# astroHaoPeng/gp_algos

Hardware: NVIDIA B200
Metric: MLE objective+gradient evals/sec at n=8192 D=8 (FP64) (higher is better)
Workload: dtype f64

## Files before the change

### gp_algos_b200/csrc/gpk_chol.cu

```cuda
#include "gpk_internal.cuh"

#include <stdlib.h>

namespace {

constexpr int NB = GPK_TILE;

struct Ctx {
    gpk_handle h;
    int64_t ld;
    int keep_L;
    int* info;
    int batch;
    int64_t sM;
    int64_t sT;
    int side_base;
};

int side_min() {
    static int v = -1;
    if (v < 0) { const char* e = getenv("GPK_SIDE_MIN"); v = e ? atoi(e) : 256; }
    return v;
}

// ... 254 lines not shown
                g.Q = Li + b1 + (int64_t)bk * N; g.ldq = N; g.q_kcontig = 0;
                g.D = rhsB + b1; g.ldd = N; g.Cin = g.D; g.ldc = N;
                g.R = rhsM; g.S = N - b1; g.K = sk; g.alpha = -1.0; g.beta = 1.0;
                rc = gpk_gemm(h, g);
                if (rc) return rc;
            }
        }
    }
    cudaEvent_t e1 = next_event(h), e2 = next_event(h);
    GPK_CUDA(h, cudaEventRecord(e1, S));
    GPK_CUDA(h, cudaStreamWaitEvent(M, e1, 0));
    GPK_CUDA(h, cudaEventRecord(e2, S1));
    GPK_CUDA(h, cudaStreamWaitEvent(M, e2, 0));
    if (rhsB) {
        cudaEvent_t e3 = next_event(h);
        GPK_CUDA(h, cudaEventRecord(e3, R));
        GPK_CUDA(h, cudaStreamWaitEvent(M, e3, 0));
    }
    tr.dump();
    return GPK_OK;
}

}

size_t gpk_chol_scratch_doubles(int N) {
    const size_t rec = rec_scratch_doubles(N);
    const size_t pipe = rec_scratch_doubles(pipe_nb()) + (size_t)pipe_nb() * N;
    const size_t fact = rec_scratch_doubles(potrf_nb_max());
    const size_t m = rec > pipe ? rec : pipe;
    return m > fact ? m : fact;
}

int gpk_potrf_inv_pipelined(gpk_handle h, double* A, double* Li, double* Kinv, double* T, int N, int keep_L, int* info_dev,
                            cudaEvent_t* kinv_done) {
    const int nbk = pipe_nb();
    const int nt = (N + nbk - 1) / nbk;
    auto bs = [&](int k) { return k * nbk < N ? k * nbk : N; };
    GPK_CUDA(h, cudaMemsetAsync(info_dev, 0, sizeof(int), h->stream));
    Ctx c{h, N, keep_L, info_dev, 1, (int64_t)N * N, 0, 0};
    double* Tdiag = T;
    double* Trow = T + rec_scratch_doubles(nbk);
    cudaStream_t M = h->stream, S = h->pipe[0], S2 = h->pipe[1], S3 = h->pipe[2];
    cudaEvent_t ev = next_event(h);
    GPK_CUDA(h, cudaEventRecord(ev, M));
    GPK_CUDA(h, cudaStreamWaitEvent(S, ev, 0));
    GPK_CUDA(h, cudaStreamWaitEvent(S2, ev, 0));
    if (Kinv) GPK_CUDA(h, cudaStreamWaitEvent(S3, ev, 0));
    cudaEvent_t evGcol_prev = nullptr;
    cudaEvent_t evLi = nullptr;
    int rc;
    Trace tr;
    tr.start(M);
    for (int k = 0; k < nt; ++k) {
        const int bk = bs(k), sk = bs(k + 1) - bk;
        rc = potrf_inv_rec(c, A + bk + (int64_t)bk * N, Li + bk + (int64_t)bk * N, Tdiag, sk, bk, 0);
        if (rc) return rc;
        cudaEvent_t evF = next_event(h);
        GPK_CUDA(h, cudaEventRecord(evF, M));
        tr.mark(M, "M:F", k);
        if (k + 1 < nt) {
            const int b1 = bs(k + 1), s1 = bs(k + 2) - b1;
            rc = stage_panel(h, A, Li, N, bk, sk, b1, N, keep_L);
            if (rc) return rc;
            cudaEvent_t evE = next_event(h);
            GPK_CUDA(h, cudaEventRecord(evE, M));
            if (evGcol_prev) GPK_CUDA(h, cudaStreamWaitEvent(M, evGcol_prev, 0));
            tr.mark(M, "M:P", k);
            rc = stage_update(h, A, Li, N, bk, sk, b1, s1, b1, N - b1, 1);
            if (rc) return rc;
            tr.mark(M, "M:Ucol", k);
            evGcol_prev = nullptr;
            if (k + 2 < nt) {
                GPK_CUDA(h, cudaStreamWaitEvent(S, evE, 0));
                StreamSwap sw(h, S);
                const int b2 = bs(k + 2), s2 = bs(k + 3) - b2;
                rc = stage_update(h, A, Li, N, bk, sk, b2, s2, b2, N - b2, 1);
                if (rc) return rc;
                evGcol_prev = next_event(h);
                GPK_CUDA(h, cudaEventRecord(evGcol_prev, S));
                if (k + 3 < nt) {
                    const int b3 = bs(k + 3);
                    rc = stage_update(h, A, Li, N, bk, sk, b3, N - b3, b3, N - b3, 1);
                    if (rc) return rc;
                }
                tr.mark(S, "S:U", k);
// ... 138 lines not shown
```

### gp_algos_b200/csrc/gpk_cov.cu

```cuda
#include "gpk_internal.cuh"

#include <stdarg.h>

namespace {

constexpr int CT = 64;
constexpr int DC = 8;
constexpr int TLD = CT + 1;

enum { MODE_SYM_FULL = 0, MODE_SYM_LOWER_PAD = 1, MODE_CROSS = 2 };

struct CovArgs {
    const double* X1; int64_t ldx1; int m;
    const double* X2; int64_t ldx2; int n;
    double* K; int64_t ldk;
    int mp, np;
    int64_t strideX1, strideX2, strideK;
    const ProblemParams* pp;
    CovParams cp;
};

__device__ __forceinline__ void store2(double* p, double a, double b, bool ok0, bool ok1) {
    if (ok0 && ok1 && ((reinterpret_cast<uintptr_t>(p) & 15) == 0)) {
        *reinterpret_cast<double2*>(p) = make_double2(a, b);
    } else {
        if (ok0) p[0] = a;
        if (ok1) p[1] = b;
    }
}

template <int MODE, int KIND>
__global__ void __launch_bounds__(256) cov_se_ard_kernel(const CovArgs a0) {
    struct View { const double* X1; const double* X2; double* K; int64_t ldx1, ldx2, ldk; int m, n, mp, np; const CovParams& cp; };
    const int64_t bz = blockIdx.z;
    const View a = {a0.X1 + bz * a0.strideX1, a0.X2 + bz * a0.strideX2, a0.K + bz * a0.strideK, a0.ldx1, a0.ldx2, a0.ldk,
                    a0.m, a0.n, a0.mp, a0.np, a0.pp ? a0.pp[bz].cp : a0.cp};
    __shared__ double xi[DC][CT];
    __shared__ double xj[DC][CT];
    __shared__ double tbuf[(MODE == MODE_SYM_FULL) ? CT * TLD : 1];

    const int bi = blockIdx.x, bj = blockIdx.y;
    if (MODE == MODE_SYM_FULL && bj > bi) return;
    if (MODE == MODE_SYM_LOWER_PAD && (bj >> 1) > (bi >> 1)) return;
    const int i0 = bi * CT, j0 = bj * CT;
    const int tid = threadIdx.x, tx = tid & 31, ty = tid >> 5;
    const int D = a.cp.D;

    double r[2][8];
#pragma unroll
    for (int q = 0; q < 2; ++q)
#pragma unroll
        for (int b = 0; b < 8; ++b) r[q][b] = 0.0;

    for (int d0 = 0; d0 < D; d0 += DC) {
        const int dc = min(DC, D - d0);
        __syncthreads();
        for (int e = tid; e < dc * CT; e += 256) {
            const int d = e / CT, l = e % CT;
            const int gi = i0 + l, gj = j0 + l;
            xi[d][l] = (gi < a.m) ? a.X1[gi + (int64_t)(d0 + d) * a.ldx1] : 0.0;
            xj[d][l] = (gj < a.n) ? a.X2[gj + (int64_t)(d0 + d) * a.ldx2] : 0.0;
        }
        __syncthreads();
        for (int d = 0; d < dc; ++d) {
            const double inv = a.cp.inv_ls2[d0 + d];
            const double x0 = xi[d][2 * tx], x1 = xi[d][2 * tx + 1];
#pragma unroll
            for (int b = 0; b < 8; ++b) {
                const double xv = xj[d][ty + 8 * b];
                const double f0 = __dsub_rn(x0, xv), f1 = __dsub_rn(x1, xv);
                if (KIND == GPK_KERNEL_CO2) {
                    r[0][b] = f0; r[1][b] = f1;
                } else {
                    r[0][b] = __dadd_rn(r[0][b], __dmul_rn(__dmul_rn(f0, inv), f0));
                    r[1][b] = __dadd_rn(r[1][b], __dmul_rn(__dmul_rn(f1, inv), f1));
                }
            }
        }
    }

    const int gi0 = i0 + 2 * tx;
#pragma unroll
    for (int b = 0; b < 8; ++b) {
        const int gj = j0 + ty + 8 * b;
        double v[2];
#pragma unroll
        for (int q = 0; q < 2; ++q) {
            const int gi = gi0 + q;
            double val;
            if (KIND == GPK_KERNEL_CO2) {
                Co2Terms t;
                val = co2_value(a.cp.inv_ls2, r[q][b], t);
            } else {
                val = __dmul_rn(a.cp.sf2, exp(__dmul_rn(-0.5, r[q][b])));
            }
            if (MODE != MODE_CROSS && gi == gj) {
                val = __dadd_rn(val, a.cp.sn2);
                if (a.cp.extra_diag != 0.0) val = __dadd_rn(val, a.cp.extra_diag);
            }
            if (gi >= a.m || gj >= a.n) val = (MODE == MODE_SYM_LOWER_PAD && gi == gj) ? 1.0 : 0.0;
            v[q] = val;
        }
        store2(a.K + gi0 + (int64_t)gj * a.ldk, v[0], v[1], gi0 < a.mp && gj < a.np, gi0 + 1 < a.mp && gj < a.np);
        if (MODE == MODE_SYM_FULL) {
            tbuf[(2 * tx) * TLD + ty + 8 * b] = v[0];
            tbuf[(2 * tx + 1) * TLD + ty + 8 * b] = v[1];
        }
    }
    if (MODE == MODE_SYM_FULL && bi != bj) {
        __syncthreads();
        const int jl0 = 2 * tx;
#pragma unroll
        for (int b = 0; b < 8; ++b) {
            const int il = ty + 8 * b;
            const int grow = j0 + jl0, gcol = i0 + il;
            store2(a.K + grow + (int64_t)gcol * a.ldk, tbuf[il * TLD + jl0], tbuf[il * TLD + jl0 + 1],
                   grow < a.n && gcol < a.m, grow + 1 < a.n && gcol < a.m);
        }
    }
}

__global__ void cov_deriv_kernel(int param_num, const double* X, int n, int64_t ldx, CovParams cp, double sf, double sn,
                                 double ls_d, double* dK, int64_t ldk) {
    const int i = blockIdx.y * blockDim.x + threadIdx.x;
    const int j = blockIdx.x;
    if (i >= n || j >= n) return;
    const int D = cp.D;
    if (cp.kind == GPK_KERNEL_CO2) {
        Co2Terms t;
        double dk[GPK_CO2_NPARAMS];
        co2_value(cp.inv_ls2, __dsub_rn(X[i], X[j]), t);
        co2_derivs(cp.inv_ls2, t, dk);
        dk[10] = (i == j) ? 2 * cp.inv_ls2[10] : 0.0;
        dK[i + (int64_t)j * ldk] = dk[param_num - 1];
        return;
    }
// ... 33 lines not shown
        out->gscale[1 + d] = 0.5 * (sf * sf) / (l * l * l);
    }
    out->gscale[D + 1] = sn;
    return GPK_OK;
}

int gpk_make_cov_params(gpk_handle h, const double* theta, int D, int has_sigma_noise, double sigma_noise, CovParams* out) {
    if (D < 1 || D > GPK_MAX_D) return gpk_set_error(h, GPK_EINVAL, "feature dimension D=%d outside 1..%d", D, GPK_MAX_D);
    memset(out, 0, sizeof(*out));
    out->D = D;
    out->kind = h ? h->kernel_family : GPK_KERNEL_SE_ARD;
    if (out->kind == GPK_KERNEL_CO2) {
        if (D != 1) return gpk_set_error(h, GPK_EINVAL, "requirement failed: This kernel is applicable only for 1D objects");
        double* par = out->inv_ls2;
        for (int p = 0; p < GPK_CO2_NPARAMS; ++p) par[p] = theta[p];
        par[11] = pow(theta[1], -3); par[12] = pow(theta[3], -3); par[13] = pow(theta[4], -3); par[14] = pow(theta[6], -3);
        par[15] = pow(theta[9], -3);
        out->sf2 = ((theta[0] * theta[0] + theta[2] * theta[2]) + theta[5] * theta[5]) + theta[8] * theta[8];
        out->sn2 = theta[10] * theta[10];
        out->extra_diag = has_sigma_noise ? sigma_noise : 0.0;
        return GPK_OK;
    }
    out->sf2 = theta[0] * theta[0];
    out->sn2 = theta[D + 1] * theta[D + 1];
    out->extra_diag = has_sigma_noise ? sigma_noise : 0.0;
    for (int d = 0; d < D; ++d) out->inv_ls2[d] = 1.0 / (theta[1 + d] * theta[1 + d]);
    return GPK_OK;
}

int gpk_cov_sym_full(gpk_handle h, const double* dX, int n, int64_t ldx, const CovParams& cp, double* dK, int64_t ldk) {
    if (n <= 0) return GPK_OK;
    CovArgs a;
    a.X1 = dX; a.ldx1 = ldx; a.m = n; a.X2 = dX; a.ldx2 = ldx; a.n = n; a.K = dK; a.ldk = ldk; a.mp = n; a.np = n; a.cp = cp;
    a.strideX1 = a.strideX2 = a.strideK = 0; a.pp = nullptr;
    const int t = (n + CT - 1) / CT;
    if (cp.kind == GPK_KERNEL_CO2) cov_se_ard_kernel<MODE_SYM_FULL, GPK_KERNEL_CO2><<<dim3(t, t), 256, 0, h->stream>>>(a);
    else cov_se_ard_kernel<MODE_SYM_FULL, GPK_KERNEL_SE_ARD><<<dim3(t, t), 256, 0, h->stream>>>(a);
    GPK_LAUNCH_CHECK(h);
    return GPK_OK;
}

int gpk_cov_sym_lower_padded(gpk_handle h, const double* dX, int n, int64_t ldx, const CovParams& cp, double* dK, int N,
                             int batch, int64_t strideX, const ProblemParams* pp_dev) {
    CovArgs a;
    a.X1 = dX; a.ldx1 = ldx; a.m = n; a.X2 = dX; a.ldx2 = ldx; a.n = n; a.K = dK; a.ldk = N; a.mp = N; a.np = N; a.cp = cp;
    a.strideX1 = a.strideX2 = strideX; a.strideK = (int64_t)N * N; a.pp = pp_dev;
    const int t = N / CT;
    if (cp.kind == GPK_KERNEL_CO2) cov_se_ard_kernel<MODE_SYM_LOWER_PAD, GPK_KERNEL_CO2><<<dim3(t, t, batch), 256, 0, h->stream>>>(a);
    else cov_se_ard_kernel<MODE_SYM_LOWER_PAD, GPK_KERNEL_SE_ARD><<<dim3(t, t, batch), 256, 0, h->stream>>>(a);
    GPK_LAUNCH_CHECK(h);
    return GPK_OK;
}

int gpk_cov_cross(gpk_handle h, const double* dX1, int m, int64_t ldx1, const double* dX2, int n, int64_t ldx2,
                  const CovParams& cp, double* dK, int64_t ldk, int mp, int np, int batch, int64_t strideX1, int64_t strideX2,
                  int64_t strideK, const ProblemParams* pp_dev) {
    if (mp < m) mp = m;
    if (np < n) np = n;
    if (mp <= 0 || np <= 0) return GPK_OK;
    CovArgs a;
    a.X1 = dX1; a.ldx1 = ldx1; a.m = m; a.X2 = dX2; a.ldx2 = ldx2; a.n = n; a.K = dK; a.ldk = ldk; a.mp = mp; a.np = np; a.cp = cp;
    a.strideX1 = strideX1; a.strideX2 = strideX2; a.strideK = strideK; a.pp = pp_dev;
    const dim3 grid((mp + CT - 1) / CT, (np + CT - 1) / CT, batch);
    if (cp.kind == GPK_KERNEL_CO2) cov_se_ard_kernel<MODE_CROSS, GPK_KERNEL_CO2><<<grid, 256, 0, h->stream>>>(a);
    else cov_se_ard_kernel<MODE_CROSS, GPK_KERNEL_SE_ARD><<<grid, 256, 0, h->stream>>>(a);
    GPK_LAUNCH_CHECK(h);
    return GPK_OK;
}

int gpk_cov_deriv(gpk_handle h, int param_num, const double* dX, int n, int64_t ldx, const CovParams& cp, double sf,
                  double sn, const double* ls_host, double* dK, int64_t ldk) {
    if (n <= 0) return GPK_OK;
    const double ls_d = (param_num >= 2 && param_num < cp.D + 2) ? ls_host[param_num - 2] : 1.0;
    cov_deriv_kernel<<<dim3(n, (n + 127) / 128), 128, 0, h->stream>>>(param_num, dX, n, ldx, cp, sf, sn, ls_d, dK, ldk);
    GPK_LAUNCH_CHECK(h);
    return GPK_OK;
}
```

### gp_algos_b200/csrc/gpk_gp.cu

```cuda
#include "gpk_internal.cuh"

#include <stdlib.h>

#include <new>

namespace {

#define ARENA_OR_FAIL(ptr, type, h, which, bytes)           \
    type ptr = (type)gpk_arena((h), (which), (bytes));      \
    if (!ptr) return GPK_ENOMEM

size_t batch_budget_bytes() {
    static size_t v = 0;
    if (!v) {
        const char* e = getenv("GPK_BATCH_GB");
        v = (size_t)((e ? atof(e) : 48.0) * (1ull << 30));
    }
    return v;
}

struct Work {
    int N, B;
    double *A, *Li, *T, *ypad, *z, *alpha, *scratch;
    size_t sT, sScratch;
// ... 23 lines not shown
    double* m = (double*)gpk_arena(h, ARENA_MISC, (size_t)B * ((size_t)3 * N + sScr) * sizeof(double));
    w->pp_dev = (ProblemParams*)gpk_arena(h, ARENA_PP, (size_t)B * sizeof(ProblemParams));
    w->info_dev = (int*)gpk_arena(h, ARENA_INFO, (size_t)B * sizeof(int));
    if (!w->A || !w->Li || !w->T || !m || !w->pp_dev || !w->info_dev) return GPK_ENOMEM;
    w->ypad = m;
    w->z = m + (size_t)B * N;
    w->alpha = m + (size_t)2 * B * N;
    w->scratch = m + (size_t)3 * B * N;
    return GPK_OK;
}

int stage_params(gpk_handle h, const double* thetas, int D, int has_s, double s, int B, ProblemParams* dev, ProblemParams* first) {
    const size_t bytes = (size_t)B * sizeof(ProblemParams);
    if (h->pp_host_bytes < bytes) {
        free(h->pp_host);
        h->pp_host = malloc(bytes);
        h->pp_host_bytes = h->pp_host ? bytes : 0;
        if (!h->pp_host) return gpk_set_error(h, GPK_ENOMEM, "host allocation failed");
    }
    ProblemParams* hp = (ProblemParams*)h->pp_host;
    for (int b = 0; b < B; ++b) {
        int rc = gpk_make_problem_params(h, thetas + (size_t)b * gpk_theta_len(h, D), D, has_s, s, &hp[b]);
        if (rc) return rc;
    }
    *first = hp[0];
    if (B > 1) {
        GPK_CUDA(h, cudaMemcpyAsync(dev, hp, bytes, cudaMemcpyHostToDevice, h->stream));
    }
    return GPK_OK;
}

int fit_core(gpk_handle h, const Work& w, int B, const double* dX, int n, int D, int64_t ldx, int64_t strideX, const double* dy,
             const ProblemParams& pp0, int keep_L, double* Li, double* alpha, double* ll_dev, int64_t ll_stride, int* info_dev,
             double* Kinv = nullptr, cudaEvent_t* kinv_done = nullptr, bool params_on_device = false) {
    const ProblemParams* ppd = (B > 1 || params_on_device) ? w.pp_dev : nullptr;
    int rc = gpk_cov_sym_lower_padded(h, dX, n, ldx, pp0.cp, w.A, w.N, B, strideX, ppd);
    if (rc) return rc;
    rc = Kinv ? gpk_potrf_inv_pipelined(h, w.A, Li, Kinv, w.T, w.N, keep_L, info_dev, kinv_done)
              : gpk_potrf_inv(h, w.A, Li, w.T, w.N, keep_L, info_dev, B);
    if (rc) return rc;
    rc = gpk_pad_vector(h, w.ypad, w.N, dy, n, B);
    if (rc) return rc;
    rc = gpk_trmv_lower(h, Li, w.N, w.ypad, w.z, w.scratch, B);
    if (rc) return rc;
    rc = gpk_trmv_lower_t(h, Li, w.N, w.z, alpha, B);
    if (rc) return rc;
    return gpk_loglik(h, w.A, w.N, n, w.ypad, alpha, ll_dev, B, ll_stride);
}

int nll_grad_core(gpk_handle h, int B, const double* dX, int n, int D, int64_t ldx, int64_t strideX, const double* dy,
                  const double* thetas, int has_s, double s, int nparams, double* out_dev, int* info_dev,
                  const ProblemParams* pp_single = nullptr) {
    Work w;
    int rc = make_work(h, n, D, B, &w);
    if (rc) return rc;
    const int64_t so = nparams + 1;
    const bool on_dev = pp_single != nullptr;
    for (int b0 = 0; b0 < B; b0 += w.B) {
        const int bc = (B - b0 < w.B) ? B - b0 : w.B;
        ProblemParams pp0;
        if (on_dev) pp0 = *pp_single;
        else rc = stage_params(h, thetas + (size_t)b0 * gpk_theta_len(h, D), D, has_s, s, bc, w.pp_dev, &pp0);
        if (rc) return rc;
        const double* X = dX + b0 * strideX;
        int* info = info_dev ? info_dev + b0 : (B == 1 ? h->d_info : w.info_dev);
        double* Kinv = nullptr;
        if (nparams > 0 && gpk_use_pipelined(w.N, bc)) {
            Kinv = (double*)gpk_arena(h, ARENA_KINV, (size_t)w.N * w.N * sizeof(double));
            if (!Kinv) return GPK_ENOMEM;
        }
        cudaEvent_t kinv_done = nullptr;
        rc = fit_core(h, w, bc, X, n, D, ldx, strideX, dy + (size_t)b0 * n, pp0, 0, w.Li, w.alpha, out_dev + b0 * so, so, info, Kinv,
                      &kinv_done, on_dev);
        if (rc) return rc;
        if (kinv_done) GPK_CUDA(h, cudaStreamWaitEvent(h->stream, kinv_done, 0));
        if (nparams > 0) {
            if (!Kinv) {
                rc = gpk_lauum_lower(h, w.Li, w.A, w.N, bc);
                if (rc) return rc;
            }
            rc = gpk_grad_trace(h, Kinv ? Kinv : w.A, w.N, X, n, ldx, w.alpha, pp0, nparams, out_dev + b0 * so + 1, w.scratch, bc, strideX,
                                (bc > 1 || on_dev) ? w.pp_dev : nullptr, so);
            if (rc) return rc;
        }
    }
    return GPK_OK;
}

__global__ void store_params_kernel(const ProblemParams pp, ProblemParams* __restrict__ dst) {
    if (threadIdx.x == 0) *dst = pp;
}

int nll_grad_single(gpk_handle h, const double* dX, int n, int D, int64_t ldx, const double* dy, const double* theta, int has_s,
                    double s, int nparams, double* out_dev, int* info_dev) {
    if (!h->graph_mode) return nll_grad_core(h, 1, dX, n, D, ldx, 0, dy, theta, has_s, s, nparams, out_dev, info_dev);
    ProblemParams pp;
    int rc = gpk_make_problem_params(h, theta, D, has_s, s, &pp);
    if (rc) return rc;
    Work w;
    rc = make_work(h, n, D, 1, &w);
    if (rc) return rc;
    if (nparams > 0 && gpk_use_pipelined(w.N, 1) && !gpk_arena(h, ARENA_KINV, (size_t)w.N * w.N * sizeof(double))) return GPK_ENOMEM;
    GraphKey key;
    memset(&key, 0, sizeof(key));
    key.p[0] = dX; key.p[1] = dy; key.p[2] = out_dev; key.p[3] = info_dev;
    key.i[0] = n; key.i[1] = D; key.i[2] = nparams; key.i[3] = ldx; key.i[4] = h->kernel_family;
    store_params_kernel<<<1, 32, 0, h->stream>>>(pp, w.pp_dev);
    GPK_LAUNCH_CHECK(h);
    auto body = [&]() { return nll_grad_core(h, 1, dX, n, D, ldx, 0, dy, theta, has_s, s, nparams, out_dev, info_dev, &pp); };
    static int after = -1;
    if (after < 0) { const char* e = getenv("GPK_GRAPH_AFTER_EVAL"); after = e ? atoi(e) : 1; if (after < 1) after = 1; }
    return gpk_graph_run(h, GPK_SLOT_EVAL, key, after, body, "evaluation");
}


__global__ void __launch_bounds__(256) ucb_grad_kernel(const double* __restrict__ KsT, const double* __restrict__ U, int N, int n,
                                                       const double* __restrict__ X, int ldx, const double* __restrict__ Xs, int ms,
                                                       const double* __restrict__ alpha, const double* __restrict__ colsq,
                                                       const double* __restrict__ mean, CovParams cp, double kparam,
                                                       double* __restrict__ grad, double* __restrict__ ucb, double* __restrict__ var) {
    __shared__ double sa[256], sb[256];
    const int c = blockIdx.x, d = blockIdx.y;
    const double xd = Xs[c + (int64_t)d * ms], inv = cp.inv_ls2[d];
    const double* ks = KsT + (int64_t)c * N;
    const double* u = U + (int64_t)c * N;
    const double* xcol = X + (int64_t)d * ldx;
    double a = 0.0, b = 0.0;
    for (int i = threadIdx.x; i < n; i += 256) {
        const double g = ((xd - xcol[i]) * inv) * (-ks[i]);
        a += g * alpha[i];
        b += g * u[i];
    }
    sa[threadIdx.x] = a; sb[threadIdx.x] = b;
    __syncthreads();
    for (int s = 128; s > 0; s >>= 1) {
// ... 546 lines not shown
```

### gp_algos_b200/csrc/gpk_grad.cu

```cuda
#include "gpk_internal.cuh"

namespace {

constexpr int GT = 64;
constexpr int GC = 8;

struct GradArgs {
    const double* Kinv; int N;
    const double* X; int64_t ldx; int n;
    const double* alpha;
    double* partial;
    int64_t strideX;
    const ProblemParams* pp;
    CovParams cp;
};

__device__ __forceinline__ double block_sum(double v, double* red) {
#pragma unroll
    for (int o = 16; o > 0; o >>= 1) v += __shfl_xor_sync(0xffffffffu, v, o);
    const int w = threadIdx.x >> 5, l = threadIdx.x & 31;
    __syncthreads();
    if (l == 0) red[w] = v;
    __syncthreads();
    double s = 0.0;
    if (threadIdx.x == 0)
        for (int i = 0; i < 8; ++i) s += red[i];
    return s;
}

__global__ void __launch_bounds__(256) grad_trace_kernel(const GradArgs a) {
    extern __shared__ double sm[];
    __shared__ double red[8];
    const int64_t pb = blockIdx.y;
    const CovParams& cp = a.pp ? a.pp[pb].cp : a.cp;
    const double* Kinv = a.Kinv ? a.Kinv + pb * (int64_t)a.N * a.N : nullptr;
    const double* X = a.X + pb * a.strideX;
    const double* alpha = a.alpha + pb * a.N;
    const int D = cp.D;
    double* xi = sm;
    double* xj = sm + D * GT;
    const int t = blockIdx.x;
    int bi = (int)((sqrt(8.0 * (double)t + 1.0) - 1.0) * 0.5);
    while ((int64_t)(bi + 1) * (bi + 2) / 2 <= t) ++bi;
    while ((int64_t)bi * (bi + 1) / 2 > t) --bi;
    const int bj = t - (int)((int64_t)bi * (bi + 1) / 2);
    const int i0 = bi * GT, j0 = bj * GT;
    const int tid = threadIdx.x, tx = tid & 31, ty = tid >> 5;

    for (int e = tid; e < D * GT; e += 256) {
        const int d = e / GT, l = e % GT;
        const int gi = i0 + l, gj = j0 + l;
        xi[e] = (gi < a.n) ? X[gi + (int64_t)d * a.ldx] : 0.0;
        xj[e] = (gj < a.n) ? X[gj + (int64_t)d * a.ldx] : 0.0;
    }
    __syncthreads();

    const int gi0 = i0 + 2 * tx;
    double we[2][8];
    double wdiag = 0.0;
    {
        double r[2][8];
#pragma unroll
        for (int q = 0; q < 2; ++q)
#pragma unroll
            for (int b = 0; b < 8; ++b) r[q][b] = 0.0;
        for (int d = 0; d < D; ++d) {
            const double inv = cp.inv_ls2[d];
            const double x0 = xi[d * GT + 2 * tx], x1 = xi[d * GT + 2 * tx + 1];
#pragma unroll
            for (int b = 0; b < 8; ++b) {
                const double xv = xj[d * GT + ty + 8 * b];
                const double f0 = x0 - xv, f1 = x1 - xv;
                r[0][b] += (f0 * inv) * f0;
                r[1][b] += (f1 * inv) * f1;
            }
        }
        const double al0 = (gi0 < a.n) ? alpha[gi0] : 0.0, al1 = (gi0 + 1 < a.n) ? alpha[gi0 + 1] : 0.0;
#pragma unroll
        for (int b = 0; b < 8; ++b) {
            const int gj = j0 + ty + 8 * b;
            const double aj = (gj < a.n) ? alpha[gj] : 0.0;
            const double2 kv = Kinv ? *reinterpret_cast<const double2*>(Kinv + gi0 + (int64_t)gj * a.N) : make_double2(0.0, 0.0);
#pragma unroll
            for (int q = 0; q < 2; ++q) {
                const int gi = gi0 + q;
                const double w = (q ? al1 : al0) * aj - (q ? kv.y : kv.x);
                const bool valid = gi < a.n && gj < a.n && gi >= gj;
                const double mult = (gi == gj) ? 1.0 : 2.0;
                we[q][b] = valid ? mult * w * exp(-0.5 * r[q][b]) : 0.0;
                if (valid && gi == gj) wdiag += w;
            }
        }
    }

    double* out = a.partial + (pb * gridDim.x + blockIdx.x) * (int64_t)(D + 2);
    {
        double s = 0.0;
#pragma unroll
        for (int q = 0; q < 2; ++q)
#pragma unroll
            for (int b = 0; b < 8; ++b) s += we[q][b];
        const double ts = block_sum(s, red);
        const double tn = block_sum(wdiag, red);
        if (tid == 0) { out[0] = ts; out[D + 1] = tn; }
    }
    for (int d0 = 0; d0 < D; d0 += GC) {
        double acc[GC];
#pragma unroll
        for (int c = 0; c < GC; ++c) acc[c] = 0.0;
#pragma unroll
        for (int c = 0; c < GC; ++c) {
            const int d = d0 + c;
            if (d < D) {
                const double x0 = xi[d * GT + 2 * tx], x1 = xi[d * GT + 2 * tx + 1];
#pragma unroll
                for (int b = 0; b < 8; ++b) {
                    const double xv = xj[d * GT + ty + 8 * b];
                    const double f0 = x0 - xv, f1 = x1 - xv;
                    acc[c] += we[0][b] * (f0 * f0) + we[1][b] * (f1 * f1);
                }
            }
        }
// ... 57 lines not shown
    }
}

struct GradScale { double s[GPK_MAX_D + 2]; };
__global__ void __launch_bounds__(256) grad_finish_kernel(const double* partial, int nblocks, int np_all, int nparams,
                                                          const GradScale scale, const ProblemParams* pp, double* g,
                                                          int64_t strideOut) {
    __shared__ double sd[256];
    const int p = blockIdx.x;
    const int64_t pb = blockIdx.y;
    if (p >= nparams) return;
    partial += pb * (int64_t)nblocks * np_all;
    double s = 0.0;
    for (int b = threadIdx.x; b < nblocks; b += 256) s += partial[(int64_t)b * np_all + p];
    sd[threadIdx.x] = s;
    __syncthreads();
    for (int k = 128; k > 0; k >>= 1) {
        if (threadIdx.x < k) sd[threadIdx.x] += sd[threadIdx.x + k];
        __syncthreads();
    }
    if (threadIdx.x == 0) g[pb * strideOut + p] = (pp ? pp[pb].gscale[p] : scale.s[p]) * sd[0];
}

}

size_t gpk_grad_scratch_doubles(int N, int D) {
    const size_t tiles = (size_t)(N / GT) * (N / GT + 1) / 2;
    const size_t np = (size_t)(D + 2 > GPK_CO2_NPARAMS ? D + 2 : GPK_CO2_NPARAMS);
    return tiles * np + np;
}

int gpk_grad_trace(gpk_handle h, const double* Kinv, int N, const double* dX, int n, int64_t ldx, const double* alpha,
                   const ProblemParams& pp, int nparams, double* g_out, double* scratch, int batch, int64_t strideX,
                   const ProblemParams* pp_dev, int64_t strideOut) {
    const int D = pp.cp.D;
    const int np_all = pp.cp.kind == GPK_KERNEL_CO2 ? GPK_CO2_NPARAMS : D + 2;
    if (nparams < 0 || nparams > np_all) return gpk_set_error(h, GPK_EINVAL, "nparams=%d outside 0..%d", nparams, np_all);
    if (nparams == 0) return GPK_OK;
    const int nt = (n + GT - 1) / GT;
    const int nblocks = nt * (nt + 1) / 2;
    GradArgs a;
    a.Kinv = Kinv; a.N = N; a.X = dX; a.ldx = ldx; a.n = n; a.alpha = alpha; a.partial = scratch; a.cp = pp.cp;
    a.strideX = strideX; a.pp = pp_dev;
    const size_t smem = (size_t)2 * D * GT * sizeof(double);
    if (smem > 48 * 1024 && !(h->func_cfg & (1u << 9))) {
        GPK_CUDA(h, cudaFuncSetAttribute(grad_trace_kernel, cudaFuncAttributeMaxDynamicSharedMemorySize,
                                         (int)((size_t)2 * GPK_MAX_D * GT * sizeof(double))));
        h->func_cfg |= (1u << 9);
    }
    if (pp.cp.kind == GPK_KERNEL_CO2) grad_trace_co2_kernel<<<dim3(nblocks, batch), 256, 0, h->stream>>>(a);
    else grad_trace_kernel<<<dim3(nblocks, batch), 256, smem, h->stream>>>(a);
    GPK_LAUNCH_CHECK(h);
    GradScale sc;
    memcpy(sc.s, pp.gscale, sizeof(sc.s));
    grad_finish_kernel<<<dim3(nparams, batch), 256, 0, h->stream>>>(scratch, nblocks, np_all, nparams, sc, pp_dev, g_out, strideOut);
    GPK_LAUNCH_CHECK(h);
    return GPK_OK;
}
```

### gp_algos_b200/csrc/gpk_internal.cuh

```cuda
#pragma once
#include <cuda_runtime.h>
#include <stdint.h>
#include <stdio.h>
#include <string.h>

#include <functional>

#include "../../include/gpk.h"

#define GPK_TILE 128
#define GPK_NPIPE 3
#define GPK_NSIDE 16
#define GPK_NGROUP 4
#define GPK_NEVENTS 256

struct gpk_handle_s {
    int device;
    cudaStream_t stream;
    cudaStream_t main_stream;
    int num_sms;
    bool own_stream;
    cudaStream_t side[GPK_NSIDE];
    cudaStream_t grp[GPK_NGROUP - 1];
    cudaStream_t pipe[GPK_NPIPE];
// ... 5 lines not shown
    void* res_pinned;
    size_t res_pinned_bytes;
    int* d_info;
    int last_info;
    int64_t launches;
    unsigned func_cfg;
    void* pp_host;
    size_t pp_host_bytes;
    int graph_mode;
    unsigned arena_epoch;
    struct gpk_graph_slot* slots[3];
    struct gpk_capture_log* cap;
    int prio_main, prio_side, prio_pipe;
    int kernel_family;
    char err[512];
};
struct StreamSwap {
    gpk_handle h; cudaStream_t saved;
    StreamSwap(gpk_handle h_, cudaStream_t s) : h(h_), saved(h_->stream) { h->stream = s; }
    ~StreamSwap() { h->stream = saved; }
};
static inline cudaEvent_t next_event(gpk_handle h) { return h->evpool[h->ev_next++ % GPK_NEVENTS]; }
#define GPK_NSLOTS 3
enum { GPK_SLOT_EVAL = 0, GPK_SLOT_EP_SWEEP = 1, GPK_SLOT_POTRF = 2 };
struct GraphKey { const void* p[6]; int64_t i[6]; };
void gpk_capture_note(gpk_handle h);
void gpk_graph_drop_all(gpk_handle h);
int gpk_graph_run_impl(gpk_handle h, int slot, const GraphKey& key, int eager_calls, int (*body)(void*), void* ctx, const char* what);
template <class F>
int gpk_graph_run(gpk_handle h, int slot, const GraphKey& key, int eager_calls, F& body, const char* what) {
    return gpk_graph_run_impl(h, slot, key, eager_calls, [](void* c) { return (*static_cast<F*>(c))(); }, &body, what);
}

enum { ARENA_A = 0, ARENA_B = 1, ARENA_T = 2, ARENA_MISC = 3, ARENA_X = 4, ARENA_IO = 5, ARENA_IO2 = 6, ARENA_IO3 = 7, ARENA_PP = 8, ARENA_INFO = 9, ARENA_GEMV = 10, ARENA_KINV = 11, GPK_NARENA = 12 };

int gpk_set_error(gpk_handle h, int status, const char* fmt, ...);
void* gpk_arena(gpk_handle h, int which, size_t bytes);
int gpk_upload_matrix(gpk_handle h, double* dst, const double* src, int rows, int cols, int64_t ld);
int gpk_download_matrix(gpk_handle h, double* dst, int64_t ld, const double* src, int rows, int cols);
int gpk_finish_info(gpk_handle h);

#define GPK_CUDA(h, call)                                                                         \
    do {                                                                                          \
        cudaError_t e__ = (call);                                                                 \
        if (e__ != cudaSuccess)                                                                   \
            return gpk_set_error((h), e__ == cudaErrorMemoryAllocation ? GPK_ENOMEM : GPK_ECUDA,  \
                                 "%s failed: %s (%s:%d)", #call, cudaGetErrorString(e__), __FILE__, __LINE__); \
    } while (0)

#define GPK_LAUNCH_CHECK(h)                                                                       \
    do {                                                                                          \
        (h)->launches++;                                                                          \
        if ((h)->cap) gpk_capture_note(h);                                                        \
        cudaError_t e__ = cudaGetLastError();                                                     \
        if (e__ != cudaSuccess)                                                                   \
            return gpk_set_error((h), GPK_ECUDA, "kernel launch failed: %s (%s:%d)",              \
                                 cudaGetErrorString(e__), __FILE__, __LINE__);                    \
    } while (0)

static inline int gpk_pad(int n) { return (n + GPK_TILE - 1) / GPK_TILE * GPK_TILE; }

struct GemmDesc {
    const double* P; int64_t ldp; int64_t strideP;
    const double* Q; int64_t ldq; int64_t strideQ;
    double* D; int64_t ldd; int64_t strideD;
    const double* Cin; int64_t ldc; int64_t strideC;
    int R, S, K;
// ... 55 lines not shown
    const double first = exp(__dmul_rn(-hp8, lg));
    const double den = __dmul_rn(__dmul_rn(__dmul_rn(__dmul_rn(__dmul_rn(2.0, hp7), hp7), hp8), hp8), t.p1);
    const double second = __dadd_rn(-lg, __dmul_rn(hp8, t.sq) / den);
    dk[7] = __dmul_rn(__dmul_rn(__dmul_rn(hp6, hp6), first), second);
    dk[8] = __dmul_rn(2.0, t.k4) / hp9;
    dk[9] = __dmul_rn(__dmul_rn(t.k4, t.sq), par[15]);
}
#endif
struct ProblemParams {
    CovParams cp;
    double gscale[GPK_MAX_D + 2];
};
int gpk_make_cov_params(gpk_handle h, const double* theta, int D, int has_sigma_noise, double sigma_noise, CovParams* out);
int gpk_make_problem_params(gpk_handle h, const double* theta, int D, int has_sigma_noise, double sigma_noise, ProblemParams* out);

struct gpk_model_s {
    int n, N, D;
    int ldx;
    double* X;
    double* Li;
    double* alpha;
    double theta[GPK_MAX_D + 2];
    ProblemParams pp;
    int has_s;
    double s;
};

int gpk_posterior(gpk_handle h, const double* dX, int n, int64_t ldx, const double* dXs, int ms, const double* Li,
                  const double* alpha, int N, const CovParams& cp, double* KsT, double* mean, double* V, int nv, double* vsq,
                  int batch = 1, int64_t strideX = 0, int64_t strideXs = 0, const ProblemParams* pp_dev = nullptr);

int gpk_cov_sym_full(gpk_handle h, const double* dX, int n, int64_t ldx, const CovParams& cp, double* dK, int64_t ldk);
int gpk_cov_sym_lower_padded(gpk_handle h, const double* dX, int n, int64_t ldx, const CovParams& cp, double* dK, int N,
                             int batch = 1, int64_t strideX = 0, const ProblemParams* pp_dev = nullptr);
int gpk_cov_cross(gpk_handle h, const double* dX1, int m, int64_t ldx1, const double* dX2, int n, int64_t ldx2,
                  const CovParams& cp, double* dK, int64_t ldk, int mp, int np, int batch = 1, int64_t strideX1 = 0,
                  int64_t strideX2 = 0, int64_t strideK = 0, const ProblemParams* pp_dev = nullptr);
int gpk_cov_deriv(gpk_handle h, int param_num, const double* dX, int n, int64_t ldx, const CovParams& cp,
                  double sf, double sn, const double* ls_host, double* dK, int64_t ldk);

int gpk_base_potrf_trtri(gpk_handle h, double* A, int64_t lda, double* Li, int64_t ldi, int* info, int col_offset, int mode,
                         int batch, int64_t strideA, int64_t strideLi, int info_stride, int coloff_stride);
size_t gpk_chol_scratch_doubles(int N);
int gpk_potrf_inv(gpk_handle h, double* A, double* Li, double* T, int N, int keep_L, int* info_dev, int batch = 1);
bool gpk_use_pipelined(int N, int batch);
int gpk_potrf_inv_pipelined(gpk_handle h, double* A, double* Li, double* Kinv, double* T, int N, int keep_L, int* info_dev,
                            cudaEvent_t* kinv_done = nullptr);
typedef std::function<int(int row0, int rows, cudaEvent_t ready)> GpkRowsHook;
int gpk_potrf_factor_solve(gpk_handle h, double* A, double* Li, double* T, int N, int* info_dev, double* B, double* V, int M,
                           const GpkRowsHook* on_rows = nullptr);
int gpk_potrf_factor(gpk_handle h, double* A, double* Li, double* T, int N, int* info_dev);
int gpk_trsm_padded(gpk_handle h, const double* Lw, double* Di, int N, int backward, double* B, double* X, int M);
int gpk_trtri_lower(gpk_handle h, const double* L, double* Li, double* T, int N);
int gpk_lauum_lower(gpk_handle h, const double* Li, double* Kinv, int N, int batch = 1);
int gpk_trmm_lower(gpk_handle h, const double* Li, int N, const double* B, double* V, int M, int batch = 1);

size_t gpk_trmv_scratch_doubles(int N);
int gpk_trmv_lower(gpk_handle h, const double* Li, int N, const double* y, double* z, double* scratch, int batch = 1);
int gpk_trmv_lower_t(gpk_handle h, const double* Li, int N, const double* z, double* a, int batch = 1);
int gpk_colwise_dot(gpk_handle h, const double* M, int64_t ld, int rows, int cols, const double* v, double* out, int square,
                    int batch = 1, int64_t strideM = 0, int64_t strideV = 0, int64_t strideOut = 0);
int gpk_gemv(gpk_handle h, int trans, int m, int ncols, double alpha, const double* M, int64_t ld, const double* x, double beta,
             double* y);
int gpk_add_diag(gpk_handle h, double* A, int64_t ld, int n, double v);
int gpk_sum_log_diag(gpk_handle h, const double* A, int64_t ld, int n, double* out, int accumulate);
int gpk_loglik(gpk_handle h, const double* A, int N, int n, const double* y, const double* alpha, double* out, int batch = 1,
               int64_t strideOut = 0);
int gpk_grad_trace(gpk_handle h, const double* Kinv, int N, const double* dX, int n, int64_t ldx, const double* alpha,
                   const ProblemParams& pp, int nparams, double* g_out, double* scratch, int batch = 1, int64_t strideX = 0,
                   const ProblemParams* pp_dev = nullptr, int64_t strideOut = 0);
size_t gpk_grad_scratch_doubles(int N, int D);

int gpk_copy2d(gpk_handle h, double* dst, int64_t ldd, const double* src, int64_t lds, int rows, int cols);
int gpk_pad_vector(gpk_handle h, double* dst, int N, const double* src, int n, int batch = 1);
int gpk_load_sym_padded(gpk_handle h, double* dst, int N, const double* src, int n, int64_t lds, int* d_notsym);
int gpk_store_lower(gpk_handle h, double* dst, int64_t ldd, const double* src, int N, int n);
int gpk_store_tri(gpk_handle h, double* dst, int64_t ldd, const double* src, int N, int n, int transpose);
int gpk_load_tri_padded(gpk_handle h, double* dst, int N, const double* src, int n, int64_t lds, int transpose_in);
```

Before: 57.64.

## Overlap covariance build with pipelined Cholesky and cache exp terms for gradient

The covariance matrix is now built in two column ranges. The first two panels are built on the main stream and the remainder on a side stream, so the build overlaps the start of the pipelined factorization. For SE-ARD the covariance kernel also stores the unscaled exp values into a new N×N buffer, which the gradient trace kernel reads instead of recomputing distances and exponentials. This trades one extra N×N write and read plus an extra arena allocation for less FP64 exp and distance work in the gradient.

New measurement: 58.09, median of 6. No clear change (+0.8%).

```diff
diff --git a/gp_algos_b200/csrc/gpk_chol.cu b/gp_algos_b200/csrc/gpk_chol.cu
--- a/gp_algos_b200/csrc/gpk_chol.cu
+++ b/gp_algos_b200/csrc/gpk_chol.cu
@@ -310,7 +310,7 @@
 }
 
 int gpk_potrf_inv_pipelined(gpk_handle h, double* A, double* Li, double* Kinv, double* T, int N, int keep_L, int* info_dev,
-                            cudaEvent_t* kinv_done) {
+                            cudaEvent_t* kinv_done, const GpkColsBuild* build_A) {
     const int nbk = pipe_nb();
     const int nt = (N + nbk - 1) / nbk;
     auto bs = [&](int k) { return k * nbk < N ? k * nbk : N; };
@@ -319,16 +319,27 @@
     double* Tdiag = T;
     double* Trow = T + rec_scratch_doubles(nbk);
     cudaStream_t M = h->stream, S = h->pipe[0], S2 = h->pipe[1], S3 = h->pipe[2];
+    int rc;
+    Trace tr;
+    tr.start(M);
+    if (build_A) {
+        rc = (*build_A)(0, bs(2));
+        if (rc) return rc;
+        tr.mark(M, "M:A", 0);
+    }
     cudaEvent_t ev = next_event(h);
     GPK_CUDA(h, cudaEventRecord(ev, M));
     GPK_CUDA(h, cudaStreamWaitEvent(S, ev, 0));
     GPK_CUDA(h, cudaStreamWaitEvent(S2, ev, 0));
     if (Kinv) GPK_CUDA(h, cudaStreamWaitEvent(S3, ev, 0));
+    if (build_A) {
+        StreamSwap sw(h, S);
+        rc = (*build_A)(bs(2), N);
+        if (rc) return rc;
+        tr.mark(S, "S:A", 0);
+    }
     cudaEvent_t evGcol_prev = nullptr;
     cudaEvent_t evLi = nullptr;
-    int rc;
-    Trace tr;
-    tr.start(M);
     for (int k = 0; k < nt; ++k) {
         const int bk = bs(k), sk = bs(k + 1) - bk;
         rc = potrf_inv_rec(c, A + bk + (int64_t)bk * N, Li + bk + (int64_t)bk * N, Tdiag, sk, bk, 0);
diff --git a/gp_algos_b200/csrc/gpk_cov.cu b/gp_algos_b200/csrc/gpk_cov.cu
--- a/gp_algos_b200/csrc/gpk_cov.cu
+++ b/gp_algos_b200/csrc/gpk_cov.cu
@@ -16,6 +16,8 @@
     double* K; int64_t ldk;
     int mp, np;
     int64_t strideX1, strideX2, strideK;
+    int t0;
+    double* E;
     const ProblemParams* pp;
     CovParams cp;
 };
@@ -39,7 +41,8 @@
     __shared__ double xj[DC][CT];
     __shared__ double tbuf[(MODE == MODE_SYM_FULL) ? CT * TLD : 1];
 
-    const int bi = blockIdx.x, bj = blockIdx.y;
+    const int t0 = (MODE == MODE_SYM_LOWER_PAD) ? a0.t0 : 0;
+    const int bi = blockIdx.x + t0, bj = blockIdx.y + t0;
     if (MODE == MODE_SYM_FULL && bj > bi) return;
     if (MODE == MODE_SYM_LOWER_PAD && (bj >> 1) > (bi >> 1)) return;
     const int i0 = bi * CT, j0 = bj * CT;
@@ -83,7 +86,7 @@
 #pragma unroll
     for (int b = 0; b < 8; ++b) {
         const int gj = j0 + ty + 8 * b;
-        double v[2];
+        double v[2], e[2] = {0.0, 0.0};
 #pragma unroll
         for (int q = 0; q < 2; ++q) {
             const int gi = gi0 + q;
@@ -92,7 +95,8 @@
                 Co2Terms t;
                 val = co2_value(a.cp.inv_ls2, r[q][b], t);
             } else {
-                val = __dmul_rn(a.cp.sf2, exp(__dmul_rn(-0.5, r[q][b])));
+                e[q] = exp(__dmul_rn(-0.5, r[q][b]));
+                val = __dmul_rn(a.cp.sf2, e[q]);
             }
             if (MODE != MODE_CROSS && gi == gj) {
                 val = __dadd_rn(val, a.cp.sn2);
@@ -102,6 +106,8 @@
             v[q] = val;
         }
         store2(a.K + gi0 + (int64_t)gj * a.ldk, v[0], v[1], gi0 < a.mp && gj < a.np, gi0 + 1 < a.mp && gj < a.np);
+        if (MODE == MODE_SYM_LOWER_PAD && KIND == GPK_KERNEL_SE_ARD && a0.E != nullptr)
+            store2(a0.E + gi0 + (int64_t)gj * a.ldk, e[0], e[1], gi0 < a.mp && gj < a.np, gi0 + 1 < a.mp && gj < a.np);
         if (MODE == MODE_SYM_FULL) {
             tbuf[(2 * tx) * TLD + ty + 8 * b] = v[0];
             tbuf[(2 * tx + 1) * TLD + ty + 8 * b] = v[1];
@@ -201,7 +207,7 @@
     if (n <= 0) return GPK_OK;
     CovArgs a;
     a.X1 = dX; a.ldx1 = ldx; a.m = n; a.X2 = dX; a.ldx2 = ldx; a.n = n; a.K = dK; a.ldk = ldk; a.mp = n; a.np = n; a.cp = cp;
-    a.strideX1 = a.strideX2 = a.strideK = 0; a.pp = nullptr;
+    a.strideX1 = a.strideX2 = a.strideK = 0; a.pp = nullptr; a.t0 = 0; a.E = nullptr;
     const int t = (n + CT - 1) / CT;
     if (cp.kind == GPK_KERNEL_CO2) cov_se_ard_kernel<MODE_SYM_FULL, GPK_KERNEL_CO2><<<dim3(t, t), 256, 0, h->stream>>>(a);
     else cov_se_ard_kernel<MODE_SYM_FULL, GPK_KERNEL_SE_ARD><<<dim3(t, t), 256, 0, h->stream>>>(a);
@@ -210,13 +216,16 @@
 }
 
 int gpk_cov_sym_lower_padded(gpk_handle h, const double* dX, int n, int64_t ldx, const CovParams& cp, double* dK, int N,
-                             int batch, int64_t strideX, const ProblemParams* pp_dev) {
+                             int batch, int64_t strideX, const ProblemParams* pp_dev, int c0, int c1, double* dE) {
+    if (c1 < 0) c1 = N;
+    if (c1 <= c0) return GPK_OK;
     CovArgs a;
     a.X1 = dX; a.ldx1 = ldx; a.m = n; a.X2 = dX; a.ldx2 = ldx; a.n = n; a.K = dK; a.ldk = N; a.mp = N; a.np = N; a.cp = cp;
-    a.strideX1 = a.strideX2 = strideX; a.strideK = (int64_t)N * N; a.pp = pp_dev;
-    const int t = N / CT;
-    if (cp.kind == GPK_KERNEL_CO2) cov_se_ard_kernel<MODE_SYM_LOWER_PAD, GPK_KERNEL_CO2><<<dim3(t, t, batch), 256, 0, h->stream>>>(a);
-    else cov_se_ard_kernel<MODE_SYM_LOWER_PAD, GPK_KERNEL_SE_ARD><<<dim3(t, t, batch), 256, 0, h->stream>>>(a);
+    a.strideX1 = a.strideX2 = strideX; a.strideK = (int64_t)N * N; a.pp = pp_dev; a.t0 = c0 / CT;
+    a.E = (batch == 1 && cp.kind == GPK_KERNEL_SE_ARD) ? dE : nullptr;
+    const dim3 grid((N - c0) / CT, (c1 - c0) / CT, batch);
+    if (cp.kind == GPK_KERNEL_CO2) cov_se_ard_kernel<MODE_SYM_LOWER_PAD, GPK_KERNEL_CO2><<<grid, 256, 0, h->stream>>>(a);
+    else cov_se_ard_kernel<MODE_SYM_LOWER_PAD, GPK_KERNEL_SE_ARD><<<grid, 256, 0, h->stream>>>(a);
     GPK_LAUNCH_CHECK(h);
     return GPK_OK;
 }
@@ -229,7 +238,7 @@
     if (mp <= 0 || np <= 0) return GPK_OK;
     CovArgs a;
     a.X1 = dX1; a.ldx1 = ldx1; a.m = m; a.X2 = dX2; a.ldx2 = ldx2; a.n = n; a.K = dK; a.ldk = ldk; a.mp = mp; a.np = np; a.cp = cp;
-    a.strideX1 = strideX1; a.strideX2 = strideX2; a.strideK = strideK; a.pp = pp_dev;
+    a.strideX1 = strideX1; a.strideX2 = strideX2; a.strideK = strideK; a.pp = pp_dev; a.t0 = 0; a.E = nullptr;
     const dim3 grid((mp + CT - 1) / CT, (np + CT - 1) / CT, batch);
     if (cp.kind == GPK_KERNEL_CO2) cov_se_ard_kernel<MODE_CROSS, GPK_KERNEL_CO2><<<grid, 256, 0, h->stream>>>(a);
     else cov_se_ard_kernel<MODE_CROSS, GPK_KERNEL_SE_ARD><<<grid, 256, 0, h->stream>>>(a);
diff --git a/gp_algos_b200/csrc/gpk_gp.cu b/gp_algos_b200/csrc/gpk_gp.cu
--- a/gp_algos_b200/csrc/gpk_gp.cu
+++ b/gp_algos_b200/csrc/gpk_gp.cu
@@ -79,12 +79,19 @@
 
 int fit_core(gpk_handle h, const Work& w, int B, const double* dX, int n, int D, int64_t ldx, int64_t strideX, const double* dy,
              const ProblemParams& pp0, int keep_L, double* Li, double* alpha, double* ll_dev, int64_t ll_stride, int* info_dev,
-             double* Kinv = nullptr, cudaEvent_t* kinv_done = nullptr, bool params_on_device = false) {
+             double* Kinv = nullptr, cudaEvent_t* kinv_done = nullptr, bool params_on_device = false, double* E = nullptr) {
     const ProblemParams* ppd = (B > 1 || params_on_device) ? w.pp_dev : nullptr;
-    int rc = gpk_cov_sym_lower_padded(h, dX, n, ldx, pp0.cp, w.A, w.N, B, strideX, ppd);
-    if (rc) return rc;
-    rc = Kinv ? gpk_potrf_inv_pipelined(h, w.A, Li, Kinv, w.T, w.N, keep_L, info_dev, kinv_done)
-              : gpk_potrf_inv(h, w.A, Li, w.T, w.N, keep_L, info_dev, B);
+    int rc;
+    if (Kinv) {
+        const GpkColsBuild build = [&](int c0, int c1) {
+            return gpk_cov_sym_lower_padded(h, dX, n, ldx, pp0.cp, w.A, w.N, B, strideX, ppd, c0, c1, E);
+        };
+        rc = gpk_potrf_inv_pipelined(h, w.A, Li, Kinv, w.T, w.N, keep_L, info_dev, kinv_done, &build);
+    } else {
+        rc = gpk_cov_sym_lower_padded(h, dX, n, ldx, pp0.cp, w.A, w.N, B, strideX, ppd);
+        if (rc) return rc;
+        rc = gpk_potrf_inv(h, w.A, Li, w.T, w.N, keep_L, info_dev, B);
+    }
     if (rc) return rc;
     rc = gpk_pad_vector(h, w.ypad, w.N, dy, n, B);
     if (rc) return rc;
@@ -112,13 +119,18 @@
         const double* X = dX + b0 * strideX;
         int* info = info_dev ? info_dev + b0 : (B == 1 ? h->d_info : w.info_dev);
         double* Kinv = nullptr;
+        double* E = nullptr;
         if (nparams > 0 && gpk_use_pipelined(w.N, bc)) {
             Kinv = (double*)gpk_arena(h, ARENA_KINV, (size_t)w.N * w.N * sizeof(double));
             if (!Kinv) return GPK_ENOMEM;
+            if (pp0.cp.kind == GPK_KERNEL_SE_ARD) {
+                E = (double*)gpk_arena(h, ARENA_E, (size_t)w.N * w.N * sizeof(double));
+                if (!E) return GPK_ENOMEM;
+            }
         }
         cudaEvent_t kinv_done = nullptr;
         rc = fit_core(h, w, bc, X, n, D, ldx, strideX, dy + (size_t)b0 * n, pp0, 0, w.Li, w.alpha, out_dev + b0 * so, so, info, Kinv,
-                      &kinv_done, on_dev);
+                      &kinv_done, on_dev, E);
         if (rc) return rc;
         if (kinv_done) GPK_CUDA(h, cudaStreamWaitEvent(h->stream, kinv_done, 0));
         if (nparams > 0) {
@@ -127,7 +139,7 @@
                 if (rc) return rc;
             }
             rc = gpk_grad_trace(h, Kinv ? Kinv : w.A, w.N, X, n, ldx, w.alpha, pp0, nparams, out_dev + b0 * so + 1, w.scratch, bc, strideX,
-                                (bc > 1 || on_dev) ? w.pp_dev : nullptr, so);
+                                (bc > 1 || on_dev) ? w.pp_dev : nullptr, so, E);
             if (rc) return rc;
         }
     }
@@ -147,7 +159,10 @@
     Work w;
     rc = make_work(h, n, D, 1, &w);
     if (rc) return rc;
-    if (nparams > 0 && gpk_use_pipelined(w.N, 1) && !gpk_arena(h, ARENA_KINV, (size_t)w.N * w.N * sizeof(double))) return GPK_ENOMEM;
+    if (nparams > 0 && gpk_use_pipelined(w.N, 1)) {
+        if (!gpk_arena(h, ARENA_KINV, (size_t)w.N * w.N * sizeof(double))) return GPK_ENOMEM;
+        if (h->kernel_family == GPK_KERNEL_SE_ARD && !gpk_arena(h, ARENA_E, (size_t)w.N * w.N * sizeof(double))) return GPK_ENOMEM;
+    }
     GraphKey key;
     memset(&key, 0, sizeof(key));
     key.p[0] = dX; key.p[1] = dy; key.p[2] = out_dev; key.p[3] = info_dev;
diff --git a/gp_algos_b200/csrc/gpk_grad.cu b/gp_algos_b200/csrc/gpk_grad.cu
--- a/gp_algos_b200/csrc/gpk_grad.cu
+++ b/gp_algos_b200/csrc/gpk_grad.cu
@@ -13,6 +13,7 @@
     int64_t strideX;
     const ProblemParams* pp;
     CovParams cp;
+    const double* E;
 };
 
 __device__ __forceinline__ double block_sum(double v, double* red) {
@@ -28,6 +29,7 @@
     return s;
 }
 
+template <bool HAS_E>
 __global__ void __launch_bounds__(256) grad_trace_kernel(const GradArgs a) {
     extern __shared__ double sm[];
     __shared__ double red[8];
@@ -64,7 +66,7 @@
         for (int q = 0; q < 2; ++q)
 #pragma unroll
             for (int b = 0; b < 8; ++b) r[q][b] = 0.0;
-        for (int d = 0; d < D; ++d) {
+        for (int d = 0; d < (HAS_E ? 0 : D); ++d) {
             const double inv = cp.inv_ls2[d];
             const double x0 = xi[d * GT + 2 * tx], x1 = xi[d * GT + 2 * tx + 1];
 #pragma unroll
@@ -81,13 +83,15 @@
             const int gj = j0 + ty + 8 * b;
             const double aj = (gj < a.n) ? alpha[gj] : 0.0;
             const double2 kv = Kinv ? *reinterpret_cast<const double2*>(Kinv + gi0 + (int64_t)gj * a.N) : make_double2(0.0, 0.0);
+            const double2 ev = HAS_E ? *reinterpret_cast<const double2*>(a.E + gi0 + (int64_t)gj * a.N) : make_double2(0.0, 0.0);
 #pragma unroll
             for (int q = 0; q < 2; ++q) {
                 const int gi = gi0 + q;
                 const double w = (q ? al1 : al0) * aj - (q ? kv.y : kv.x);
                 const bool valid = gi < a.n && gj < a.n && gi >= gj;
                 const double mult = (gi == gj) ? 1.0 : 2.0;
-                we[q][b] = valid ? mult * w * exp(-0.5 * r[q][b]) : 0.0;
+                const double e = HAS_E ? (q ? ev.y : ev.x) : exp(-0.5 * r[q][b]);
+                we[q][b] = valid ? mult * w * e : 0.0;
                 if (valid && gi == gj) wdiag += w;
             }
         }
@@ -211,7 +215,7 @@
 
 int gpk_grad_trace(gpk_handle h, const double* Kinv, int N, const double* dX, int n, int64_t ldx, const double* alpha,
                    const ProblemParams& pp, int nparams, double* g_out, double* scratch, int batch, int64_t strideX,
-                   const ProblemParams* pp_dev, int64_t strideOut) {
+                   const ProblemParams* pp_dev, int64_t strideOut, const double* E) {
     const int D = pp.cp.D;
     const int np_all = pp.cp.kind == GPK_KERNEL_CO2 ? GPK_CO2_NPARAMS : D + 2;
     if (nparams < 0 || nparams > np_all) return gpk_set_error(h, GPK_EINVAL, "nparams=%d outside 0..%d", nparams, np_all);
@@ -220,15 +224,17 @@
     const int nblocks = nt * (nt + 1) / 2;
     GradArgs a;
     a.Kinv = Kinv; a.N = N; a.X = dX; a.ldx = ldx; a.n = n; a.alpha = alpha; a.partial = scratch; a.cp = pp.cp;
-    a.strideX = strideX; a.pp = pp_dev;
+    a.strideX = strideX; a.pp = pp_dev; a.E = E;
+    if (E && (batch != 1 || pp.cp.kind != GPK_KERNEL_SE_ARD)) return gpk_set_error(h, GPK_EINVAL, "gpk_grad_trace: E needs one SE-ARD problem");
     const size_t smem = (size_t)2 * D * GT * sizeof(double);
     if (smem > 48 * 1024 && !(h->func_cfg & (1u << 9))) {
-        GPK_CUDA(h, cudaFuncSetAttribute(grad_trace_kernel, cudaFuncAttributeMaxDynamicSharedMemorySize,
-                                         (int)((size_t)2 * GPK_MAX_D * GT * sizeof(double))));
+        for (auto k : {grad_trace_kernel<false>, grad_trace_kernel<true>})
+            GPK_CUDA(h, cudaFuncSetAttribute(k, cudaFuncAttributeMaxDynamicSharedMemorySize, (int)((size_t)2 * GPK_MAX_D * GT * sizeof(double))));
         h->func_cfg |= (1u << 9);
     }
     if (pp.cp.kind == GPK_KERNEL_CO2) grad_trace_co2_kernel<<<dim3(nblocks, batch), 256, 0, h->stream>>>(a);
-    else grad_trace_kernel<<<dim3(nblocks, batch), 256, smem, h->stream>>>(a);
+    else if (E) grad_trace_kernel<true><<<dim3(nblocks, batch), 256, smem, h->stream>>>(a);
+    else grad_trace_kernel<false><<<dim3(nblocks, batch), 256, smem, h->stream>>>(a);
     GPK_LAUNCH_CHECK(h);
     GradScale sc;
     memcpy(sc.s, pp.gscale, sizeof(sc.s));
diff --git a/gp_algos_b200/csrc/gpk_internal.cuh b/gp_algos_b200/csrc/gpk_internal.cuh
--- a/gp_algos_b200/csrc/gpk_internal.cuh
+++ b/gp_algos_b200/csrc/gpk_internal.cuh
@@ -61,7 +61,7 @@
     return gpk_graph_run_impl(h, slot, key, eager_calls, [](void* c) { return (*static_cast<F*>(c))(); }, &body, what);
 }
 
-enum { ARENA_A = 0, ARENA_B = 1, ARENA_T = 2, ARENA_MISC = 3, ARENA_X = 4, ARENA_IO = 5, ARENA_IO2 = 6, ARENA_IO3 = 7, ARENA_PP = 8, ARENA_INFO = 9, ARENA_GEMV = 10, ARENA_KINV = 11, GPK_NARENA = 12 };
+enum { ARENA_A = 0, ARENA_B = 1, ARENA_T = 2, ARENA_MISC = 3, ARENA_X = 4, ARENA_IO = 5, ARENA_IO2 = 6, ARENA_IO3 = 7, ARENA_PP = 8, ARENA_INFO = 9, ARENA_GEMV = 10, ARENA_KINV = 11, ARENA_E = 12, GPK_NARENA = 13 };
 
 int gpk_set_error(gpk_handle h, int status, const char* fmt, ...);
 void* gpk_arena(gpk_handle h, int which, size_t bytes);
@@ -183,7 +183,8 @@
 
 int gpk_cov_sym_full(gpk_handle h, const double* dX, int n, int64_t ldx, const CovParams& cp, double* dK, int64_t ldk);
 int gpk_cov_sym_lower_padded(gpk_handle h, const double* dX, int n, int64_t ldx, const CovParams& cp, double* dK, int N,
-                             int batch = 1, int64_t strideX = 0, const ProblemParams* pp_dev = nullptr);
+                             int batch = 1, int64_t strideX = 0, const ProblemParams* pp_dev = nullptr, int c0 = 0, int c1 = -1,
+                             double* dE = nullptr);
 int gpk_cov_cross(gpk_handle h, const double* dX1, int m, int64_t ldx1, const double* dX2, int n, int64_t ldx2,
                   const CovParams& cp, double* dK, int64_t ldk, int mp, int np, int batch = 1, int64_t strideX1 = 0,
                   int64_t strideX2 = 0, int64_t strideK = 0, const ProblemParams* pp_dev = nullptr);
@@ -195,8 +196,9 @@
 size_t gpk_chol_scratch_doubles(int N);
 int gpk_potrf_inv(gpk_handle h, double* A, double* Li, double* T, int N, int keep_L, int* info_dev, int batch = 1);
 bool gpk_use_pipelined(int N, int batch);
+typedef std::function<int(int c0, int c1)> GpkColsBuild;
 int gpk_potrf_inv_pipelined(gpk_handle h, double* A, double* Li, double* Kinv, double* T, int N, int keep_L, int* info_dev,
-                            cudaEvent_t* kinv_done = nullptr);
+                            cudaEvent_t* kinv_done = nullptr, const GpkColsBuild* build_A = nullptr);
 typedef std::function<int(int row0, int rows, cudaEvent_t ready)> GpkRowsHook;
 int gpk_potrf_factor_solve(gpk_handle h, double* A, double* Li, double* T, int N, int* info_dev, double* B, double* V, int M,
                            const GpkRowsHook* on_rows = nullptr);
@@ -219,7 +221,7 @@
                int64_t strideOut = 0);
 int gpk_grad_trace(gpk_handle h, const double* Kinv, int N, const double* dX, int n, int64_t ldx, const double* alpha,
                    const ProblemParams& pp, int nparams, double* g_out, double* scratch, int batch = 1, int64_t strideX = 0,
-                   const ProblemParams* pp_dev = nullptr, int64_t strideOut = 0);
+                   const ProblemParams* pp_dev = nullptr, int64_t strideOut = 0, const double* E = nullptr);
 size_t gpk_grad_scratch_doubles(int N, int D);
 
 int gpk_copy2d(gpk_handle h, double* dst, int64_t ldd, const double* src, int64_t lds, int rows, int cols);
```
